# josedelrey/genetic-gaussian-splats

Measured on AMD Instinct MI355X. Metric: candidate renders/sec (and Gsplat-pixels/s), 512x512, 256 splats, pop=128, higher is better.
Workload: dtype fp32

## Files before the change

### genetic-gaussian-splats_amd/csrc/ggs_capi.cpp

```cpp
#include <hip/hip_runtime.h>
#include <math.h>
#include <stdarg.h>
#include <stdio.h>
#include <stdlib.h>
#include <string.h>

#include <algorithm>
#include <atomic>
#include <memory>
#include <mutex>
#include <string>
#include <vector>

#include "ggs_internal.h"


namespace ggs {
namespace {

thread_local std::string t_err;

int fail(int code, const char* fmt, ...) {
    char buf[512];
    va_list ap;
// ... 36 lines not shown
    }
    const size_t want = std::max<size_t>(bytes + bytes / 4, 4096);
    GGS_HIP(hipMalloc(&b.p, want));
    b.cap = want;
    return GGS_OK;
}

int ensure_zeroed(DevBuf& b, size_t bytes, hipStream_t st) {
    if (bytes <= b.cap) return GGS_OK;
    int rc = ensure(b, bytes, st);
    if (rc) return rc;
    GGS_HIP(hipMemsetAsync(b.p, 0, b.cap, st));
    return GGS_OK;
}

bool finalize_fused() {
    static const bool off = getenv("GGS_UNFUSED_FINALIZE") && atoi(getenv("GGS_UNFUSED_FINALIZE")) != 0;
    return !off;
}
bool fitness_api_fold() {
    const char* v = getenv("GGS_FITNESS_FOLD");
    return v && atoi(v) != 0;
}

struct PinBuf {
    void* p = nullptr;
    size_t cap = 0;
};

int ensure_pinned(PinBuf& b, size_t bytes) {
    if (bytes <= b.cap) return GGS_OK;
    if (b.p) {
        GGS_HIP(hipHostFree(b.p));
        b.p = nullptr;
        b.cap = 0;
    }
    const size_t want = std::max<size_t>(bytes + bytes / 4, 4096);
    GGS_HIP(hipHostMalloc(&b.p, want, hipHostMallocDefault));
    b.cap = want;
    return GGS_OK;
}

struct Workspace {
    hipStream_t stream = nullptr;
    DevBuf recs, bnds, partials, wpartials, order, plan, fctr;
    DevBuf maskws;
    int order_H = -1, order_W = -1;
    uint64_t plan_key = 0;
};

int ensure_tile_order(Workspace* w, int H, int W, hipStream_t st) {
    if (w->order_H == H && w->order_W == W) return GGS_OK;
    const int n = raster_order_len(H, W);
    int rc;
    if ((rc = ensure(w->order, sizeof(int) * (size_t)n, st))) return rc;
    std::vector<int> h(n);
    raster_tile_order(H, W, h.data());
#ifdef GGS_PROBE_BUILD
    if (const char* f = getenv("GGS_PROBE_ORDER")) {
        FILE* fp = fopen(f, "rb");
        if (!fp || fread(h.data(), sizeof(int), n, fp) != (size_t)n) {
            if (fp) fclose(fp);
            return fail(GGS_EINVAL, "GGS_PROBE_ORDER: cannot read the order");
        }
        fclose(fp);
    }
#endif
    GGS_HIP(hipStreamSynchronize(st));
    GGS_HIP(hipMemcpy(w->order.p, h.data(), sizeof(int) * n, hipMemcpyHostToDevice));
// ... 51 lines not shown
        if (!on) return;
        (void)hipEventRecord(b, st);
        std::lock_guard<std::mutex> lk(g_prof_mu);
        g_prof_pending.push_back({kernel, a, b});
    }
};

void prof_drain_locked() {
    for (auto& r : g_prof_pending) {
        float ms = 0.f;
        if (hipEventSynchronize(r.b) == hipSuccess && hipEventElapsedTime(&ms, r.a, r.b) == hipSuccess) {
            g_prof_ms[r.kernel] += ms;
            g_prof_n[r.kernel] += 1;
        }
        (void)hipEventDestroy(r.a);
        (void)hipEventDestroy(r.b);
    }
    g_prof_pending.clear();
}

int raster_fitness(hipStream_t st, int simds, const SplatRec* recs, const int4* bnds, int B, int N, int H, int W,
                   const float4* plan, float* partials, const float* wpartials, int mode, const int* order,
                   DevBuf& ctr, float* out, bool fuse, const unsigned char* dirty = nullptr,
                   const float* clean = nullptr, int group = 0) {
    const float bg[3] = {1.f, 1.f, 1.f};
    int nTX;
    const int nTiles = raster_tiles(H, W, &nTX);
    if (fuse && finalize_fused() && (4 * nTiles) % 32 == 0) {
        int rc;
        if ((rc = ensure_zeroed(ctr, sizeof(int) * (size_t)std::max(B, 1), st))) return rc;
        FinFused ff;
        ff.ctr = (int*)ctr.p;
        ff.wpartials = wpartials;
        ff.out = out;
        ff.hw = (double)H * (double)W;
        ff.mode = mode;
        ProfScope ps(st, 1);
        GGS_HIP(launch_raster(st, 1, recs, bnds, B, N, H, W, bg, nullptr, plan, partials, order, dirty, clean,
                              nullptr, &ff, simds, group));
        return GGS_OK;
    }
    {
        ProfScope ps(st, 1);
        GGS_HIP(launch_raster(st, 1, recs, bnds, B, N, H, W, bg, nullptr, plan, partials, order, dirty, clean,
                              nullptr, nullptr, simds, group));
    }
    ProfScope ps(st, 2);
    GGS_HIP(launch_finalize(st, partials, wpartials, B, nTiles, mode, H, W, out, nullptr, group));
    return GGS_OK;
}

struct DeviceGuard {
    int prev = -1;
    explicit DeviceGuard(int dev) {
        if (hipGetDevice(&prev) != hipSuccess) prev = -1;
        (void)hipSetDevice(dev);
    }
    ~DeviceGuard() {
        if (prev >= 0) (void)hipSetDevice(prev);
    }
};

struct StreamDrain {
    std::vector<std::pair<int, hipStream_t>> s;
    void add(int dev, hipStream_t st) {
        for (auto& x : s)
            if (x.second == st) return;
        s.emplace_back(dev, st);
// ... 99 lines not shown
    h ^= h >> 33;
    h *= P2;
    h ^= h >> 29;
    h *= P3;
    h ^= h >> 32;
    return h;
}

int check_dims(int64_t B, int32_t N, int32_t C, int32_t H, int32_t W) {
    if (B < 0 || N < 0) return fail(GGS_EINVAL, "B=%lld and N=%d must be >= 0", (long long)B, N);
    if (C < 9) return fail(GGS_EINVAL, "expected at least 9 genome cols, got C=%d (render.py:223)", C);
    if (H < 1 || W < 1) return fail(GGS_EINVAL, "H=%d, W=%d must be >= 1", H, W);
    if ((int64_t)N * (int64_t)sizeof(SplatRec) >= ((int64_t)1 << 31))
        return fail(GGS_EINVAL, "N=%d splats per candidate exceeds the limit %lld", N,
                    (long long)(((int64_t)1 << 31) / (int64_t)sizeof(SplatRec) - 1));
    int nTX;
    const int64_t nTiles = raster_tiles(H, W, &nTX);
    if (B * nTiles * 4 >= (int64_t)1 << 31)
        return fail(GGS_EINVAL, "B*tiles = %lld exceeds the grid limit; split the batch",
                    (long long)(B * nTiles * 4));
    return GGS_OK;
}

int run_fitness_planned(DevCtx* c, hipStream_t st, const float* d_gen, int64_t B, int N, int C,
                        const float4* plan, const float* wpartials, int mode, int H, int W, float k,
                        float* d_out, int group = 0);

int run_fitness(DevCtx* c, hipStream_t st, const float* d_gen, int64_t B, int N, int C,
                const float* d_target, const float* d_mask, int mode, float beta, int H, int W,
                float k, float* d_out, uint64_t plan_key = 0) {
    if (B == 0) return GGS_OK;
    Workspace* w = workspace_for(c, st);
    int nTX;
    const int nTiles = raster_tiles(H, W, &nTX);
    int rc;
    if ((rc = ensure(w->recs, sizeof(SplatRec) * (size_t)std::max<int64_t>(B * N, 1), st))) return rc;
    if ((rc = ensure(w->bnds, sizeof(int4) * (size_t)std::max<int64_t>(B * N, 1), st))) return rc;
    if ((rc = ensure(w->partials, sizeof(float) * 4 * (size_t)(B * nTiles), st))) return rc;
    if ((rc = ensure(w->wpartials, plan_wsum_bytes(H, W), st))) return rc;
    if ((rc = ensure_tile_order(w, H, W, st))) return rc;
    if (plan_key == 0 || plan_key != w->plan_key) {
        if ((rc = ensure(w->plan, plan_bytes(H, W), st))) return rc;
        GGS_HIP(launch_plan(st, d_target, d_mask, mode, beta, H, W, (float4*)w->plan.p,
                            (float*)w->wpartials.p));
        w->plan_key = plan_key;
    }
    return run_fitness_planned(c, st, d_gen, B, N, C, (const float4*)w->plan.p,
                               (const float*)w->wpartials.p, mode, H, W, k, d_out);
}

int run_fitness_planned(DevCtx* c, hipStream_t st, const float* d_gen, int64_t B, int N, int C,
                        const float4* plan, const float* wpartials, int mode, int H, int W, float k,
                        float* d_out, int group) {
    if (B == 0) return GGS_OK;
    Workspace* w = workspace_for(c, st);
    int nTX;
    const int nTiles = raster_tiles(H, W, &nTX);
    int rc;
    if ((rc = ensure(w->recs, sizeof(SplatRec) * (size_t)std::max<int64_t>(B * N, 1), st))) return rc;
    if ((rc = ensure(w->bnds, sizeof(int4) * (size_t)std::max<int64_t>(B * N, 1), st))) return rc;
    if ((rc = ensure(w->partials, sizeof(float) * 4 * (size_t)(B * nTiles), st))) return rc;
    if ((rc = ensure_tile_order(w, H, W, st))) return rc;
    SplatRec* recs = (SplatRec*)w->recs.p;
    {
        ProfScope ps(st, 0);
        GGS_HIP(launch_prep(st, true, d_gen, B * N, C, H, W, k, recs, (int4*)w->bnds.p, nullptr, nullptr, nullptr));
    }
    return raster_fitness(st, c->simds, recs, (const int4*)w->bnds.p, (int)B, N, H, W, plan, (float*)w->partials.p,
                          wpartials, mode, (const int*)w->order.p, w->fctr, d_out, fitness_api_fold(), nullptr,
                          nullptr, group);
}

int run_render(DevCtx* c, hipStream_t st, const float* d_gen, int64_t B, int N, int C, int H, int W,
               float k, const float bg[3], float* d_img) {
    if (B == 0) return GGS_OK;
    Workspace* w = workspace_for(c, st);
    int rc;
    if ((rc = ensure(w->recs, sizeof(SplatRec) * (size_t)std::max<int64_t>(B * N, 1), st))) return rc;
    if ((rc = ensure(w->bnds, sizeof(int4) * (size_t)std::max<int64_t>(B * N, 1), st))) return rc;
    if ((rc = ensure_tile_order(w, H, W, st))) return rc;
    SplatRec* recs = (SplatRec*)w->recs.p;
    {
        ProfScope ps(st, 0);
        GGS_HIP(launch_prep(st, false, d_gen, B * N, C, H, W, k, recs, (int4*)w->bnds.p, nullptr, nullptr, nullptr));
    }
    {
        ProfScope ps(st, 1);
        GGS_HIP(launch_raster(st, 0, recs, (const int4*)w->bnds.p, (int)B, N, H, W, bg, d_img, nullptr, nullptr,
                              (const int*)w->order.p, nullptr, nullptr, nullptr, nullptr, c->simds));
    }
    return GGS_OK;
}

void shard(int64_t B, int n, int d, int64_t* b0, int64_t* nb) {
    const int64_t per = (B + n - 1) / n;
    *b0 = std::min<int64_t>(B, d * per);
    *nb = std::min<int64_t>(B, *b0 + per) - *b0;
}

std::vector<int> g_comm_devs;
std::vector<void*> g_comms;

int local_comms_locked(const std::vector<DevCtx*>& cs, std::vector<void*>* out) {
    std::vector<int> devs;
    for (DevCtx* c : cs) devs.push_back(c->dev);
    if (devs != g_comm_devs) {
        for (void* c : g_comms) ggs_comm_destroy(c);
        g_comms.clear();
        g_comm_devs.clear();
        std::vector<void*> made(devs.size(), nullptr);
        const int rc = ggs_comm_init_local((int32_t)devs.size(), devs.data(), made.data());
        if (rc) return rc;
// ... 44 lines not shown
}

const char* ggs_last_error(void) { return t_err.c_str(); }

void ggs_shutdown(void) {
    {
        std::lock_guard<std::mutex> cl(g_comm_mu);
        for (void* c : g_comms) ggs_comm_destroy(c);
        g_comms.clear();
        g_comm_devs.clear();
    }
    std::lock_guard<std::mutex> lk(g_mu);
    {
        std::lock_guard<std::mutex> pl(g_prof_mu);
        prof_drain_locked();
    }
    for (auto& c : g_ctx) {
        if (!c) continue;
        std::lock_guard<std::mutex> cl(c->mu);
        (void)hipSetDevice(c->dev);
        (void)hipStreamSynchronize(c->stream);
        for (auto& w : c->ws) {
            if (w->stream) (void)hipStreamSynchronize(w->stream);
            for (DevBuf* b : {&w->recs, &w->bnds, &w->partials, &w->wpartials, &w->order, &w->plan, &w->fctr, &w->maskws})
                if (b->p) (void)hipFree(b->p);
        }
        for (DevBuf* b : {&c->gen, &c->out, &c->target, &c->mask, &c->prep_in, &c->prep_tgt, &c->prep_mask})
            if (b->p) (void)hipFree(b->p);
        for (PinBuf* b : {&c->h_out})
            if (b->p) (void)hipHostFree(b->p);
        (void)hipStreamDestroy(c->stream);
    }
    g_ctx.clear();
    g_active.clear();
    g_inited = false;
}

int ggs_fitness_device(int32_t device, void* stream, const float* d_genomes_axes, int64_t B, int32_t N,
                       int32_t C, const float* d_target_hw3, const float* d_mask_hw, int32_t mode,
                       float boost_beta, int32_t H, int32_t W, float k_sigma, float* d_out_B) {
    int rc = check_dims(B, N, C, H, W);
    if (rc) return rc;
    if (mode < GGS_FIT_NONE || mode > GGS_FIT_BOOST) return fail(GGS_EINVAL, "bad fitness mode %d", mode);
    if (mode != GGS_FIT_NONE && !d_mask_hw) return fail(GGS_EINVAL, "mode %d needs a weight mask", mode);
    if (B > 0 && (!d_genomes_axes && N > 0)) return fail(GGS_EINVAL, "null genomes");
    if (B > 0 && (!d_target_hw3 || !d_out_B)) return fail(GGS_EINVAL, "null target/out");
    DevCtx* c = nullptr;
// ... 2294 lines not shown
```

### genetic-gaussian-splats_amd/csrc/ggs_internal.h

```cpp
#pragma once
#include <hip/hip_runtime.h>
#include <stdint.h>

#include "../../include/ggs.h"

#if !defined(GGS_PROBE_BUILD) &&                                                         \
    (defined(GGS_NOPLAN) || defined(GGS_TIMING) || defined(GGS_VTIMING) || defined(GGS_SATURATE) || \
     defined(GGS_SAT_EVERY) || defined(GGS_SAT_BATCH) || defined(GGS_SAT_AHEAD) ||             \
     defined(GGS_CULL_AHEAD) || defined(GGS_CHUNK_MB) || defined(GGS_NO_RATIO_CLAMP) ||               \
     defined(GGS_DEPTH_SPLIT) || defined(GGS_TILE_H))
#error "GGS_* diagnostic knobs are for the probe build only: make probe PROBE=\"-D...\""
#endif
#ifdef GGS_PROBE_BUILD
#define GGS_BUILD_KIND "probe"
#else
#define GGS_BUILD_KIND "product"
#endif

namespace ggs {

struct __attribute__((aligned(16))) SplatRec {
    float C64, cx, r, cy8;
    float g, la, b, c128;
    float rho, rho4, A, B8;
    int x0, x1, y0, y1;
};
static_assert(sizeof(SplatRec) == 64, "SplatRec must be 64 bytes");

hipError_t launch_prep(hipStream_t st, bool encode, const float* genomes, int64_t S, int C, int H,
                       int W, float k, SplatRec* recs, int4* bnds, float* f9, int* i4, float* enc9,
                       const int* live = nullptr, int n_per = 0);
int raster_tiles(int H, int W, int* nTX);
struct FinFused {
    int* ctr = nullptr;
    const float* wpartials = nullptr;
    float* out = nullptr;
    double hw = 0.0;
    int mode = 0;
};
hipError_t launch_raster(hipStream_t st, int mode, const SplatRec* recs, const int4* bnds, int B, int N, int H, int W,
                         const float bg[3], float* img, const float4* plan, float* partials,
                         const int* tile_order, const unsigned char* dirty = nullptr,
                         const float* clean = nullptr, const int* live = nullptr, const FinFused* fin = nullptr,
                         int simds = 0, int group = 0);
int device_simds(int dev);

hipError_t launch_dirty(hipStream_t st, const float* curr, const float* nb, const SplatRec* cur_recs,
                        const SplatRec* nb_recs, int n, int N, int H, int W, unsigned char* dirty,
                        unsigned* n_changed, const int* live = nullptr, int rule = 1);
hipError_t launch_plan(hipStream_t st, const float* target, const float* mask, int mode, float beta,
                       int H, int W, float4* plan, float* wblock);
hipError_t launch_plan_set(hipStream_t st, const float* targets, const float* masks, int mode, float beta,
                           int H, int W, int K, float4* plans, float* wblocks);
size_t plan_bytes(int H, int W);
size_t plan_wsum_bytes(int H, int W);
void raster_tile_order(int H, int W, int* order);
int raster_order_len(int H, int W);
hipError_t launch_detmath(hipStream_t st, const float* x, const float* y, int64_t n, int fn,
                          float* out);
hipError_t launch_finalize(hipStream_t st, const float* partials, const float* wpartials, int B,
                           int nTiles, int mode, int H, int W, float* out, const int* live = nullptr,
                           int group = 0);

struct GaParamsDev {
    float sig_xy, sig_alog, sig_blog, sig_theta, sig_rgb, sig_alpha;
    float mutpb, cxpb;
    int tour_k;
// ... 212 lines not shown
```

### genetic-gaussian-splats_amd/csrc/ggs_kernels.hip

```cpp
#include <hip/hip_runtime.h>
#include <stdint.h>

#include <algorithm>
#include <atomic>
#include <utility>
#include <vector>

#include "ggs_detmath.h"
#include "ggs_internal.h"
#include "ggs_prep.h"

#if defined(__HIP_DEVICE_COMPILE__) && !defined(__gfx950__)
#error "ggs_kernels.hip targets gfx950 (MI355X) only"
#endif

namespace ggs {

using namespace detmath;

constexpr int PREP_THREADS = 64;
template <bool ENCODE>
__global__ void __launch_bounds__(PREP_THREADS)
prep_kernel(const float* __restrict__ genomes, int64_t S, int C, int H, int W, float k,
            SplatRec* __restrict__ recs, int4* __restrict__ bnds, float* __restrict__ f9, int* __restrict__ i4,
            float* __restrict__ enc9, const int* __restrict__ live, int n_per) {
    const int64_t i = (int64_t)blockIdx.x * blockDim.x + threadIdx.x;
    if (i >= S) return;
    if (live && i >= (int64_t)*live * n_per) return;
    const float* g = genomes + i * (int64_t)C;
    float row[9];
    if (ENCODE) {
        encode_row(g, row);
    } else {
#pragma unroll
        for (int j = 0; j < 9; ++j) row[j] = g[j];
    }
    if (enc9) {
#pragma unroll
        for (int j = 0; j < 9; ++j) enc9[i * 9 + j] = row[j];
    }
    const Prep13 p = preprocess_row(row, H, W, k);
    if (recs) {
        const SplatRec r = make_rec(p);
        recs[i] = r;
        bnds[i] = rec_bounds(r);
    }
    if (f9) {
        f9[0 * S + i] = p.cx;  f9[1 * S + i] = p.cy;  f9[2 * S + i] = p.sxx;
        f9[3 * S + i] = p.sxy; f9[4 * S + i] = p.syy; f9[5 * S + i] = p.rc;
        f9[6 * S + i] = p.gc;  f9[7 * S + i] = p.bc;  f9[8 * S + i] = p.a;
    }
    if (i4) {
        i4[0 * S + i] = p.x0; i4[1 * S + i] = p.x1; i4[2 * S + i] = p.y0; i4[3 * S + i] = p.y1;
    }
}

constexpr int TILE = 64;
#ifndef GGS_TILE_H
#define GGS_TILE_H 128
#endif
constexpr int TILE_H = GGS_TILE_H;
constexpr int RG = TILE_H / 4;
constexpr int NPK = RG / 2;
constexpr int WPB = 1;
constexpr int NT = 64 * WPB;
constexpr int SPB = 4 / WPB;
constexpr int CAP = 1024;
constexpr int OCC = 3;
// ... 10 lines not shown
#define GGS_NOPLAN 0
#endif

#ifndef GGS_SATURATE
#define GGS_SATURATE 1
#endif
constexpr float SAT_EPS = 5.9604645e-8f;
#ifndef GGS_SAT_EVERY
#define GGS_SAT_EVERY 16
#endif
constexpr int SAT_FIRST = 64, SAT_EVERY = GGS_SAT_EVERY;
constexpr int SAT_MIN_SPLATS = 512;
#ifndef GGS_SAT_BATCH
#define GGS_SAT_BATCH 384
#endif
#ifndef GGS_SAT_AHEAD
#define GGS_SAT_AHEAD 2
#endif
constexpr int SAT_BATCH = GGS_SAT_BATCH;

__device__ __forceinline__ int ufirst(int v) { return __builtin_amdgcn_readfirstlane(v); }

constexpr unsigned VW_ABOVE = 32u, VW_KA = 26, VW_CLIP = 31, VW_OFFSET = 0x03FFFFC0u;
__device__ __forceinline__ int visit_word(int i, const int4& bb, int ty0, int sx0) {
    constexpr int NP = GGS_TILE_H / 8;
    const int dy0 = bb.z - ty0, dy1 = bb.w - ty0;
    const unsigned kA = (unsigned)max(dy0, 0) >> 3;
    const unsigned kB = dy1 >= GGS_TILE_H - 1 ? (unsigned)NP : (unsigned)dy1 >> 3;
    const unsigned above = dy0 <= 0 ? VW_ABOVE : 0u;
    const unsigned clip = max(bb.x - sx0, sx0 + 15 - bb.y) > 0 ? (1u << VW_CLIP) : 0u;
    return (int)(((unsigned)i << 6) | kB | above | (kA << VW_KA) | clip);
}

__device__ __forceinline__ void store_partial(float* p, float v, bool fused) {
    if (fused) __hip_atomic_store(p, v, __ATOMIC_RELAXED, __HIP_MEMORY_SCOPE_AGENT);
    else *p = v;
}
__device__ __forceinline__ void strip_done(const FinFused& fin, const float* partials, int b, int nslots,
                                           int lane) {
    int old = 0;
    if (lane == 0) {
        asm volatile("s_waitcnt vmcnt(0)" ::: "memory");
        old = __hip_atomic_fetch_add(fin.ctr + b, 1, __ATOMIC_RELAXED, __HIP_MEMORY_SCOPE_AGENT);
    }
    if (ufirst(old) != nslots - 1) return;
    __builtin_amdgcn_fence(__ATOMIC_ACQUIRE, "agent");
    const float v = finalize_wave<true>(partials, fin.wpartials, nslots, fin.mode, fin.hw, b);
    if (lane == 0) {
        fin.out[b] = v;
        __hip_atomic_store(fin.ctr + b, 0, __ATOMIC_RELAXED, __HIP_MEMORY_SCOPE_AGENT);
    }
}

#ifndef GGS_TIMING
// ... 51 lines not shown
        P_T##k = P_T##k - w_;                                                        \
    } while (0)
#define GGS_BLEND_REC(k)                                                             \
    if ((k) < NPK) {                                                                 \
        F2 = F2 * R2;                                                                \
        R2 = R2 * (f2_t)s.rho;                                                       \
        GGS_BLEND(k, F2);                                                            \
    }
#if defined(GGS_NO_RATIO_CLAMP) && GGS_NO_RATIO_CLAMP
#define GGS_RATIO(qy8) GGS_EXP2(__builtin_fmaf((qy8), s.c128, abx.y))
#else
#define GGS_RATIO(qy8) GGS_EXP2(fminf(__builtin_fmaf((qy8), s.c128, abx.y), 100.0f))
#endif
#define GGS_E1(qy) ({                                                                     \
        f2_t t_, e2_, pxu_;                                                               \
        pxu_.x = px;                                                                      \
        const uint64_t ccp_ = *reinterpret_cast<const uint64_t*>(&s.C64);                  \
        asm("v_pk_fma_f32 %0, %1, %2, %3 op_sel:[0,0,1] op_sel_hi:[0,1,1]" : "=v"(t_) : "s"(ccp_), "v"(qy), "v"(abx)); \
        asm("v_pk_fma_f32 %0, %1, %2, %3 op_sel_hi:[1,1,0]" : "=v"(e2_) : "v"(qy), "v"(t_), "v"(pxu_)); \
        e2_; })
#define GGS_FOR8(X) X(0) X(1) X(2) X(3) X(4) X(5) X(6) X(7)
#define GGS_FOR16P(X) GGS_FOR8(X) X(8) X(9) X(10) X(11) X(12) X(13) X(14) X(15)

template <int MODE, bool SAT, bool FUSED, bool MULTI, bool LIST = false>
__device__ __forceinline__ void
raster_body(const SplatRec* __restrict__ recs, const int4* __restrict__ bnds, int B, int N, int H, int W, int nTX,
            int nTiles,
            float bg_r, float bg_g, float bg_b, float* __restrict__ img,
            const float4* __restrict__ plan, float* __restrict__ partials,
            const int* __restrict__ tile_order, const unsigned char* __restrict__ dirty,
            const float* __restrict__ clean, const int* __restrict__ live, int CH, FinFused fin, int simds,
            int group, const int* __restrict__ plan_of = nullptr) {
    static_assert(!MULTI || MODE == 1, "plan sets are for the fitness epilogue");
    static_assert(!LIST || MULTI, "a plan list names plans of a plan set");
    constexpr bool DS = GGS_DEPTH_SPLIT && MODE == 1 && !SAT;
    constexpr bool VW = !SAT && !FUSED;
    __shared__ int lists[DS ? 2 : WPB][CAP];

    const int lane = threadIdx.x & 63;
#if GGS_TIMING
    const unsigned long long rt_start = __builtin_amdgcn_s_memrealtime();
    unsigned long long t_cull = 0, t_vis = 0, t_mark = __builtin_amdgcn_s_memtime();
    unsigned n_vis = 0, n_done = 0;
#endif
#if GGS_DEPTH_SPLIT
    const int wib = DS ? 0 : ufirst((int)(threadIdx.x >> 6));
    const int half = DS ? ufirst((int)(threadIdx.x >> 6)) : 0;
#else
    const int wib = ufirst((int)(threadIdx.x >> 6));
#endif
    if (live) {
        B = ufirst(*live);
        if ((int64_t)blockIdx.x >= (int64_t)B * nTiles * SPB) return;
    }
    int idx = blockIdx.x, b0 = 0, Bc = B;
// ... 54 lines not shown
#else
    int* __restrict__ list = &lists[0][0] + wib * CAP;
#define GGS_NHI N
#define GGS_NLO 0
#define GGS_NR N
#define GGS_LIST_AT(q) list[q]
#endif
    const uint64_t lt_mask = (lane == 0) ? 0ull : (~0ull >> (64 - lane));
    int cnt = 0;
    auto saturated = [&]() __attribute__((always_inline)) {
        float m = 0.0f;
#define GGS_TMAX(k) if ((k) < NPK) m = fmaxf(m, fmaxf(P_T##k.x, P_T##k.y));
        GGS_FOR16P(GGS_TMAX)
#undef GGS_TMAX
        return !__ballot(m >= SAT_EPS);
    };

    auto bounds = [&](int i) { return cbnd[max(i, 0)]; };
#ifndef GGS_CULL_AHEAD
#define GGS_CULL_AHEAD 2
#endif
    constexpr int AHEAD = SAT ? GGS_SAT_AHEAD : GGS_CULL_AHEAD;
    static_assert(AHEAD >= 1 && AHEAD <= 4, "cull prefetch depth");
    int4 bbA = bounds(GGS_NHI - 1 - lane), bbB, bbC, bbD;
    if constexpr (AHEAD > 1) { __builtin_amdgcn_sched_barrier(0); bbB = bounds(GGS_NHI - 1 - lane - 64); }
    if constexpr (AHEAD > 2) { __builtin_amdgcn_sched_barrier(0); bbC = bounds(GGS_NHI - 1 - lane - 128); }
    if constexpr (AHEAD > 3) { __builtin_amdgcn_sched_barrier(0); bbD = bounds(GGS_NHI - 1 - lane - 192); }
    int base = 0;
    constexpr int LIMIT = SAT ? SAT_BATCH - 64 : CAP - 64 * AHEAD;
    static_assert(LIMIT + 64 * AHEAD <= CAP, "cull list capacity");
#if GGS_DEPTH_SPLIT
    for (int pass = 0;; ++pass) {
        if (DS ? pass > 0 : base >= nr) break;
#else
    while (base < N) {
#endif
        __builtin_amdgcn_s_setprio(CULL_PRIO);
#define GGS_CULL_CHUNK(BB)                                                                  \
        {                                                                                   \
            const int i = GGS_NHI - 1 - (base + lane);                                      \
            const int4 bb = BB;                                                \
            if (AHEAD == 1) BB = bounds(i - 64);                                            \
            const bool hit = (i >= GGS_NLO) & (bb.w >= ty0) & (bb.z <= ty1) & (bb.y >= sx0) & (bb.x <= sx0 + 15); \
                          \
            if (AHEAD > 1) BB = bounds(i - 64 * AHEAD);                                     \
            const uint64_t m = __ballot(hit);                                               \
            if (hit) list[cnt + __popcll(m & lt_mask)] =                                    \
                VW ? visit_word(i, bb, ty0, sx0) : i * (int)sizeof(SplatRec);                \
            cnt += __popcll(m);                                                             \
            base += 64;                                                                     \
        }
        if constexpr (AHEAD == 1) {
            GGS_CULL_CHUNK(bbA)
            if (cnt <= LIMIT && base < GGS_NR) continue;
        } else {
            do {
                GGS_CULL_CHUNK(bbA)
                GGS_CULL_CHUNK(bbB)
                if constexpr (AHEAD > 2) GGS_CULL_CHUNK(bbC)
                if constexpr (AHEAD > 3) GGS_CULL_CHUNK(bbD)
            } while (cnt <= LIMIT && base < GGS_NR);
        }
#undef GGS_CULL_CHUNK
#if GGS_DEPTH_SPLIT
        if constexpr (DS) {
            static_assert(!DS || SAT_MIN_SPLATS / 2 + 64 * AHEAD <= CAP, "depth split: one cull batch");
            if (lane == 0) s_cnt[half] = cnt;
            __syncthreads();
            c0 = ufirst(s_cnt[0]);
            const int total = c0 + ufirst(s_cnt[1]), hs = (total + 1) >> 1;
            lbase = half ? hs : 0;
            cnt = half ? total - hs : hs;
        }
#endif
        if (cnt == 0) continue;
// ... 345 lines not shown
    }
#if GGS_TIMING
    {
        GGS_TMARK(now);
        const unsigned long long rt_end = __builtin_amdgcn_s_memrealtime();
        if (lane == 0 && blockIdx.x < GGS_TIMING_WAVES) {
            unsigned long long* o = g_ggs_timing + 8 * (size_t)blockIdx.x;
            o[0] = rt_start; o[1] = rt_end; o[2] = t_cull; o[3] = t_vis; o[4] = now - t_mark;
            o[5] = (unsigned long long)__builtin_amdgcn_s_getreg(0xF804) |
                   ((unsigned long long)__builtin_amdgcn_s_getreg(0xF814) << 32);
            o[6] = n_vis; o[7] = n_done;
        }
    }
#endif
}

template <int MODE, bool SAT, bool FUSED>
__global__ void __launch_bounds__(GGS_DEPTH_SPLIT ? 2 * NT : NT, OCC)
raster_kernel(const SplatRec* __restrict__ recs, const int4* __restrict__ bnds, int B, int N, int H, int W, int nTX,
              int nTiles,
              float bg_r, float bg_g, float bg_b, float* __restrict__ img,
              const float4* __restrict__ plan, float* __restrict__ partials,
              const int* __restrict__ tile_order, const unsigned char* __restrict__ dirty,
              const float* __restrict__ clean, const int* __restrict__ live, int CH, FinFused fin, int simds) {
    raster_body<MODE, SAT, FUSED, false>(recs, bnds, B, N, H, W, nTX, nTiles, bg_r, bg_g, bg_b, img, plan, partials,
                                         tile_order, dirty, clean, live, CH, fin, simds, 1);
}

template <bool SAT, bool FUSED>
__global__ void __launch_bounds__(GGS_DEPTH_SPLIT ? 2 * NT : NT, OCC)
raster_multi_kernel(const SplatRec* __restrict__ recs, const int4* __restrict__ bnds, int B, int N, int H, int W,
                    int nTX, int nTiles, float bg_r, float bg_g, float bg_b, const float4* __restrict__ plan,
                    float* __restrict__ partials, const int* __restrict__ tile_order, int CH, FinFused fin,
                    int simds, int group) {
    raster_body<1, SAT, FUSED, true>(recs, bnds, B, N, H, W, nTX, nTiles, bg_r, bg_g, bg_b, nullptr, plan, partials,
                                     tile_order, nullptr, nullptr, nullptr, CH, fin, simds, group);
}

template <bool SAT>
__global__ void __launch_bounds__(GGS_DEPTH_SPLIT ? 2 * NT : NT, OCC)
chain_strips_kernel(const SplatRec* __restrict__ recs, const int4* __restrict__ bnds, int B, int N, int H, int W,
                    int nTX, int nTiles, float bg_r, float bg_g, float bg_b, const float4* __restrict__ plan,
                    float* __restrict__ partials, const int* __restrict__ tile_order,
                    const int* __restrict__ live, int CH, int simds, const int* __restrict__ plan_of) {
    raster_body<1, SAT, false, true, true>(recs, bnds, B, N, H, W, nTX, nTiles, bg_r, bg_g, bg_b, nullptr, plan,
                                           partials, tile_order, nullptr, nullptr, live, CH, FinFused{}, simds, 1,
                                           plan_of);
}

// ... 135 lines not shown
    const float a = x[i];
    float r, s, c;
    switch (fn) {
        case 0: r = det_expf(a); break;
        case 1: r = det_logf(a); break;
        case 2: det_sincosf(a, &s, &c); r = s; break;
        case 3: det_sincosf(a, &s, &c); r = c; break;
        case 4: r = ggs_sqrt_rn(a); break;
        default: r = ggs_div_rn(a, y[i]); break;
    }
    out[i] = r;
}

hipError_t launch_detmath(hipStream_t st, const float* x, const float* y, int64_t n, int fn,
                          float* out) {
    if (n <= 0) return hipSuccess;
    hipLaunchKernelGGL(detmath_kernel, dim3((unsigned)((n + 255) / 256)), dim3(256), 0, st, x, y, n,
                       fn, out);
    return hipGetLastError();
}

hipError_t launch_prep(hipStream_t st, bool encode, const float* genomes, int64_t S, int C, int H,
                       int W, float k, SplatRec* recs, int4* bnds, float* f9, int* i4, float* enc9, const int* live,
                       int n_per) {
    if (S <= 0) return hipSuccess;
    constexpr int PB = PREP_THREADS;
    const unsigned grid = (unsigned)((S + PB - 1) / PB);
    if (encode)
        hipLaunchKernelGGL(prep_kernel<true>, dim3(grid), dim3(PB), 0, st, genomes, S, C, H, W, k,
                           recs, bnds, f9, i4, enc9, live, n_per);
    else
        hipLaunchKernelGGL(prep_kernel<false>, dim3(grid), dim3(PB), 0, st, genomes, S, C, H, W, k,
                           recs, bnds, f9, i4, enc9, live, n_per);
    return hipGetLastError();
}

void raster_tile_order(int H, int W, int* order) {
    int nTX;
    const int n = raster_tiles(H, W, &nTX) * SPB;
    std::vector<std::pair<double, int>> d(n);
    for (int g = 0; g < n; ++g) {
        const int t = g / SPB, s = g % SPB;
        const double cx = (t % nTX) * TILE + (s + 0.5) * (TILE / SPB) - 0.5 * W;
        const double cy = (t / nTX) * TILE_H + 0.5 * TILE_H - 0.5 * H;
        d[g] = {cx * cx + cy * cy, g};
    }
    std::stable_sort(d.begin(), d.end());
    for (int g = 0; g < n; ++g) order[g] = d[g].second;
}

int raster_order_len(int H, int W) { return raster_tiles(H, W, nullptr) * SPB; }

int raster_tiles(int H, int W, int* nTX) {
    const int tx = (W + TILE - 1) / TILE, ty = (H + TILE_H - 1) / TILE_H;
    if (nTX) *nTX = tx;
    return tx * ty;
}

#ifndef GGS_CHUNK_MB
#define GGS_CHUNK_MB 40
#endif
constexpr int64_t CHUNK_BYTES = (int64_t)GGS_CHUNK_MB << 20;
int raster_chunk(int N) {
    const int64_t per = (int64_t)(N > 1 ? N : 1) * (int64_t)(sizeof(SplatRec) + sizeof(int4));
    int64_t ch = CHUNK_BYTES / per;
    if (ch > (1 << 24)) ch = 1 << 24;
    ch &= ~int64_t(7);
    return ch < 8 ? 8 : (int)ch;
}

int device_simds(int dev) {
    int cus = 0;
    if (hipDeviceGetAttribute(&cus, hipDeviceAttributeMultiprocessorCount, dev) != hipSuccess) return 0;
    return 4 * cus;
}

hipError_t launch_raster(hipStream_t st, int mode, const SplatRec* recs, const int4* bnds, int B, int N, int H, int W,
                         const float bg[3], float* img, const float4* plan, float* partials,
                         const int* tile_order, const unsigned char* dirty, const float* clean,
                         const int* live, const FinFused* fin, int simds, int group) {
    int nTX;
    const int nTiles = raster_tiles(H, W, &nTX);
    const dim3 grid((unsigned)((int64_t)B * nTiles * SPB)), block(NT);
    const bool sat = N > SAT_MIN_SPLATS;
    const dim3 block_f(GGS_DEPTH_SPLIT && !sat ? 2 * NT : NT);
    const int CH = raster_chunk(N);
    const FinFused ff = (mode != 0 && fin) ? *fin : FinFused{};
    if (GGS_DEPTH_SPLIT) simds = 0;
#define GGS_RASTER(M, S, F)                                                                    \
    hipLaunchKernelGGL((raster_kernel<M, S, F>), grid, (M) ? block_f : block, 0, st, recs, bnds, B, N, H, W, nTX, nTiles, \
                       bg[0], bg[1], bg[2], img, plan, partials, tile_order, dirty, clean, live, CH, ff, simds)
#define GGS_RASTER_MULTI(S, F)                                                                 \
    hipLaunchKernelGGL((raster_multi_kernel<S, F>), grid, block_f, 0, st, recs, bnds, B, N, H, W, nTX, nTiles, bg[0], \
                       bg[1], bg[2], plan, partials, tile_order, CH, ff, simds, group)
    if (group > 0) {
        if (mode != 1 || dirty || clean || live) return hipErrorInvalidValue;
        if (!ff.ctr) { if (!sat) GGS_RASTER_MULTI(false, false); else GGS_RASTER_MULTI(true, false); }
        else { if (!sat) GGS_RASTER_MULTI(false, true); else GGS_RASTER_MULTI(true, true); }
    }
    else if (mode == 0) { if (!sat) GGS_RASTER(0, false, false); else GGS_RASTER(0, true, false); }
    else if (!ff.ctr) { if (!sat) GGS_RASTER(1, false, false); else GGS_RASTER(1, true, false); }
    else { if (!sat) GGS_RASTER(1, false, true); else GGS_RASTER(1, true, true); }
#undef GGS_RASTER_MULTI
#undef GGS_RASTER
    return hipGetLastError();
}

hipError_t launch_chain_strips(hipStream_t st, const SplatRec* recs, const int4* bnds, int B, int N, int H, int W,
                               const float4* plans, float* partials, const int* tile_order, const int* live,
                               const int* plan_of, int simds) {
    int nTX;
    const int nTiles = raster_tiles(H, W, &nTX);
    if (!live || !plan_of) return hipErrorInvalidValue;
    const bool sat = N > SAT_MIN_SPLATS;
    const dim3 grid((unsigned)((int64_t)B * nTiles * SPB)), block(GGS_DEPTH_SPLIT && !sat ? 2 * NT : NT);
    const int CH = raster_chunk(N);
    if (GGS_DEPTH_SPLIT) simds = 0;
    if (!sat)
        hipLaunchKernelGGL(chain_strips_kernel<false>, grid, block, 0, st, recs, bnds, B, N, H, W, nTX, nTiles, 1.f,
                           1.f, 1.f, plans, partials, tile_order, live, CH, simds, plan_of);
    else
        hipLaunchKernelGGL(chain_strips_kernel<true>, grid, block, 0, st, recs, bnds, B, N, H, W, nTX, nTiles, 1.f,
                           1.f, 1.f, plans, partials, tile_order, live, CH, simds, plan_of);
    return hipGetLastError();
}
// ... 16 lines not shown
```

Before: 922,600.

## Precompute per-strip visit words and hit masks in prep for raster culling

The prep kernel now also builds, for each candidate, the per-tile-row visit words plus ballot-built 64-bit bitmasks. The masks record which splats touch each 16-pixel column strip, which ones it clips, and which touch each tile row. The unfused raster kernel then builds its per-tile cull list by ANDing these masks and scattering the precomputed words. This replaces loading each splat's bounds and testing them again in every tile. The cost is extra prep work, new workspace buffers and more memory traffic for the masks. Paths it does not cover (saturated, fused, depth-split, dirty or live) go to a bounds-culling kernel instead.

```diff
diff --git a/genetic-gaussian-splats_amd/csrc/ggs_capi.cpp b/genetic-gaussian-splats_amd/csrc/ggs_capi.cpp
--- a/genetic-gaussian-splats_amd/csrc/ggs_capi.cpp
+++ b/genetic-gaussian-splats_amd/csrc/ggs_capi.cpp
@@ -82,6 +82,10 @@
     const char* v = getenv("GGS_FITNESS_FOLD");
     return v && atoi(v) != 0;
 }
+bool strip_words_on() {
+    const char* v = getenv("GGS_STRIP_WORDS");
+    return !(v && *v && atoi(v) == 0);
+}
 
 struct PinBuf {
     void* p = nullptr;
@@ -105,6 +109,7 @@
     hipStream_t stream = nullptr;
     DevBuf recs, bnds, partials, wpartials, order, plan, fctr;
     DevBuf maskws;
+    DevBuf swords, smasks;
     int order_H = -1, order_W = -1;
     uint64_t plan_key = 0;
 };
@@ -202,7 +207,7 @@
 int raster_fitness(hipStream_t st, int simds, const SplatRec* recs, const int4* bnds, int B, int N, int H, int W,
                    const float4* plan, float* partials, const float* wpartials, int mode, const int* order,
                    DevBuf& ctr, float* out, bool fuse, const unsigned char* dirty = nullptr,
-                   const float* clean = nullptr, int group = 0) {
+                   const float* clean = nullptr, int group = 0, const StripWords& sw = StripWords{}) {
     const float bg[3] = {1.f, 1.f, 1.f};
     int nTX;
     const int nTiles = raster_tiles(H, W, &nTX);
@@ -223,7 +228,7 @@
     {
         ProfScope ps(st, 1);
         GGS_HIP(launch_raster(st, 1, recs, bnds, B, N, H, W, bg, nullptr, plan, partials, order, dirty, clean,
-                              nullptr, nullptr, simds, group));
+                              nullptr, nullptr, simds, group, sw));
     }
     ProfScope ps(st, 2);
     GGS_HIP(launch_finalize(st, partials, wpartials, B, nTiles, mode, H, W, out, nullptr, group));
@@ -369,6 +374,15 @@
     return GGS_OK;
 }
 
+int ensure_strip_words(Workspace* w, int64_t B, int N, int H, int W, hipStream_t st, StripWords* sw) {
+    if (!strip_words_ok(N) || !strip_words_on()) return GGS_OK;
+    int rc;
+    if ((rc = ensure(w->swords, strip_words_bytes(B, N, H, W), st))) return rc;
+    if ((rc = ensure(w->smasks, strip_masks_bytes(B, N, H, W), st))) return rc;
+    sw->words = (int*)w->swords.p;
+    sw->masks = (uint64_t*)w->smasks.p;
+    return GGS_OK;
+}
 int run_fitness_planned(DevCtx* c, hipStream_t st, const float* d_gen, int64_t B, int N, int C,
                         const float4* plan, const float* wpartials, int mode, int H, int W, float k,
                         float* d_out, int group = 0);
@@ -409,13 +423,17 @@
     if ((rc = ensure(w->partials, sizeof(float) * 4 * (size_t)(B * nTiles), st))) return rc;
     if ((rc = ensure_tile_order(w, H, W, st))) return rc;
     SplatRec* recs = (SplatRec*)w->recs.p;
+    const bool fold = fitness_api_fold();
+    StripWords sw;
+    if (group == 0 && !fold && (rc = ensure_strip_words(w, B, N, H, W, st, &sw))) return rc;
     {
         ProfScope ps(st, 0);
-        GGS_HIP(launch_prep(st, true, d_gen, B * N, C, H, W, k, recs, (int4*)w->bnds.p, nullptr, nullptr, nullptr));
+        GGS_HIP(launch_prep(st, true, d_gen, B * N, C, H, W, k, recs, (int4*)w->bnds.p, nullptr, nullptr, nullptr,
+                            nullptr, 0, sw, N));
     }
     return raster_fitness(st, c->simds, recs, (const int4*)w->bnds.p, (int)B, N, H, W, plan, (float*)w->partials.p,
-                          wpartials, mode, (const int*)w->order.p, w->fctr, d_out, fitness_api_fold(), nullptr,
-                          nullptr, group);
+                          wpartials, mode, (const int*)w->order.p, w->fctr, d_out, fold, nullptr,
+                          nullptr, group, sw);
 }
 
 int run_render(DevCtx* c, hipStream_t st, const float* d_gen, int64_t B, int N, int C, int H, int W,
@@ -427,14 +445,17 @@
     if ((rc = ensure(w->bnds, sizeof(int4) * (size_t)std::max<int64_t>(B * N, 1), st))) return rc;
     if ((rc = ensure_tile_order(w, H, W, st))) return rc;
     SplatRec* recs = (SplatRec*)w->recs.p;
+    StripWords sw;
+    if ((rc = ensure_strip_words(w, B, N, H, W, st, &sw))) return rc;
     {
         ProfScope ps(st, 0);
-        GGS_HIP(launch_prep(st, false, d_gen, B * N, C, H, W, k, recs, (int4*)w->bnds.p, nullptr, nullptr, nullptr));
+        GGS_HIP(launch_prep(st, false, d_gen, B * N, C, H, W, k, recs, (int4*)w->bnds.p, nullptr, nullptr, nullptr,
+                            nullptr, 0, sw, N));
     }
     {
         ProfScope ps(st, 1);
         GGS_HIP(launch_raster(st, 0, recs, (const int4*)w->bnds.p, (int)B, N, H, W, bg, d_img, nullptr, nullptr,
-                              (const int*)w->order.p, nullptr, nullptr, nullptr, nullptr, c->simds));
+                              (const int*)w->order.p, nullptr, nullptr, nullptr, nullptr, c->simds, 0, sw));
     }
     return GGS_OK;
 }
@@ -525,7 +546,8 @@
         (void)hipStreamSynchronize(c->stream);
         for (auto& w : c->ws) {
             if (w->stream) (void)hipStreamSynchronize(w->stream);
-            for (DevBuf* b : {&w->recs, &w->bnds, &w->partials, &w->wpartials, &w->order, &w->plan, &w->fctr, &w->maskws})
+            for (DevBuf* b : {&w->recs, &w->bnds, &w->partials, &w->wpartials, &w->order, &w->plan, &w->fctr, &w->maskws,
+                              &w->swords, &w->smasks})
                 if (b->p) (void)hipFree(b->p);
         }
         for (DevBuf* b : {&c->gen, &c->out, &c->target, &c->mask, &c->prep_in, &c->prep_tgt, &c->prep_mask})
diff --git a/genetic-gaussian-splats_amd/csrc/ggs_internal.h b/genetic-gaussian-splats_amd/csrc/ggs_internal.h
--- a/genetic-gaussian-splats_amd/csrc/ggs_internal.h
+++ b/genetic-gaussian-splats_amd/csrc/ggs_internal.h
@@ -27,9 +27,16 @@
 };
 static_assert(sizeof(SplatRec) == 64, "SplatRec must be 64 bytes");
 
+struct StripWords {
+    int* words = nullptr;
+    uint64_t* masks = nullptr;
+};
+bool strip_words_ok(int N);
+size_t strip_words_bytes(int64_t B, int N, int H, int W);
+size_t strip_masks_bytes(int64_t B, int N, int H, int W);
 hipError_t launch_prep(hipStream_t st, bool encode, const float* genomes, int64_t S, int C, int H,
                        int W, float k, SplatRec* recs, int4* bnds, float* f9, int* i4, float* enc9,
-                       const int* live = nullptr, int n_per = 0);
+                       const int* live = nullptr, int n_per = 0, const StripWords& sw = StripWords{}, int N = 0);
 int raster_tiles(int H, int W, int* nTX);
 struct FinFused {
     int* ctr = nullptr;
@@ -42,7 +49,7 @@
                          const float bg[3], float* img, const float4* plan, float* partials,
                          const int* tile_order, const unsigned char* dirty = nullptr,
                          const float* clean = nullptr, const int* live = nullptr, const FinFused* fin = nullptr,
-                         int simds = 0, int group = 0);
+                         int simds = 0, int group = 0, const StripWords& sw = StripWords{});
 int device_simds(int dev);
 
 hipError_t launch_dirty(hipStream_t st, const float* curr, const float* nb, const SplatRec* cur_recs,
diff --git a/genetic-gaussian-splats_amd/csrc/ggs_kernels.hip b/genetic-gaussian-splats_amd/csrc/ggs_kernels.hip
--- a/genetic-gaussian-splats_amd/csrc/ggs_kernels.hip
+++ b/genetic-gaussian-splats_amd/csrc/ggs_kernels.hip
@@ -19,12 +19,15 @@
 using namespace detmath;
 
 constexpr int PREP_THREADS = 64;
+__device__ __forceinline__ void prep_strip_words(int N, int H, int W, const int4& bb,
+                                                 int* __restrict__ swords, uint64_t* __restrict__ smasks);
 template <bool ENCODE>
 __global__ void __launch_bounds__(PREP_THREADS)
 prep_kernel(const float* __restrict__ genomes, int64_t S, int C, int H, int W, float k,
             SplatRec* __restrict__ recs, int4* __restrict__ bnds, float* __restrict__ f9, int* __restrict__ i4,
-            float* __restrict__ enc9, const int* __restrict__ live, int n_per) {
-    const int64_t i = (int64_t)blockIdx.x * blockDim.x + threadIdx.x;
+            float* __restrict__ enc9, const int* __restrict__ live, int n_per,
+            int* __restrict__ swords, uint64_t* __restrict__ smasks, int N) {
+    const int64_t i = (int64_t)blockIdx.x * blockDim.x + (smasks ? 63 - (int)threadIdx.x : (int)threadIdx.x);
     if (i >= S) return;
     if (live && i >= (int64_t)*live * n_per) return;
     const float* g = genomes + i * (int64_t)C;
@@ -44,6 +47,7 @@
         const SplatRec r = make_rec(p);
         recs[i] = r;
         bnds[i] = rec_bounds(r);
+        if (smasks) prep_strip_words(N, H, W, rec_bounds(r), swords, smasks);
     }
     if (f9) {
         f9[0 * S + i] = p.cx;  f9[1 * S + i] = p.cy;  f9[2 * S + i] = p.sxx;
@@ -100,14 +104,55 @@
 __device__ __forceinline__ int ufirst(int v) { return __builtin_amdgcn_readfirstlane(v); }
 
 constexpr unsigned VW_ABOVE = 32u, VW_KA = 26, VW_CLIP = 31, VW_OFFSET = 0x03FFFFC0u;
-__device__ __forceinline__ int visit_word(int i, const int4& bb, int ty0, int sx0) {
+__device__ __forceinline__ int visit_row_word(int i, const int4& bb, int ty0) {
     constexpr int NP = GGS_TILE_H / 8;
+    static_assert(NP == NPK, "kB counts the raster's packed row pairs");
+    static_assert(NPK < 32, "kB (0..NPK) lies below VW_ABOVE");
     const int dy0 = bb.z - ty0, dy1 = bb.w - ty0;
     const unsigned kA = (unsigned)max(dy0, 0) >> 3;
     const unsigned kB = dy1 >= GGS_TILE_H - 1 ? (unsigned)NP : (unsigned)dy1 >> 3;
     const unsigned above = dy0 <= 0 ? VW_ABOVE : 0u;
-    const unsigned clip = max(bb.x - sx0, sx0 + 15 - bb.y) > 0 ? (1u << VW_CLIP) : 0u;
-    return (int)(((unsigned)i << 6) | kB | above | (kA << VW_KA) | clip);
+    return (int)(((unsigned)i << 6) | kB | above | (kA << VW_KA));
+}
+__device__ __forceinline__ bool strip_clips(const int4& bb, int sx0) { return max(bb.x - sx0, sx0 + 15 - bb.y) > 0; }
+__device__ __forceinline__ int visit_word(int i, const int4& bb, int ty0, int sx0) {
+    return visit_row_word(i, bb, ty0) | (int)(strip_clips(bb, sx0) ? 1u << VW_CLIP : 0u);
+}
+static_assert(SAT_MIN_SPLATS * sizeof(SplatRec) <= VW_OFFSET + 64, "a record offset fits the word's offset field");
+
+__host__ __device__ constexpr int strip_mask_chunks(int N) { return ((N >> 6) + 3) & ~3; }
+__device__ __forceinline__ void prep_strip_words(int N, int H, int W, const int4& bb,
+                                                 int* __restrict__ swords, uint64_t* __restrict__ smasks) {
+    const int lane = threadIdx.x;
+    const int first = (int)(blockIdx.x * 64u), b = first / N, s = first - b * N + 63 - lane;
+    const int nTY = (H + TILE_H - 1) / TILE_H, nCS = (W + TILE - 1) / TILE * 4, R = 2 * nCS + nTY;
+    const int ncp = strip_mask_chunks(N);
+    for (int ty = 0; ty < nTY; ++ty) swords[((int64_t)b * nTY + ty) * N + s] = visit_row_word(s, bb, ty * TILE_H);
+    uint64_t* __restrict__ mcol = smasks + (int64_t)b * R * ncp + ((N >> 6) - 1 - (s >> 6));
+    const int lo = bb.x >> 4, hi = bb.y >> 4, flo = (bb.x + 15) >> 4, fhi = ((bb.y + 1) >> 4) - 1;
+    const int nW = (W + 15) >> 4;
+    for (int c0 = 0; c0 < nCS; c0 += 64) {
+        uint64_t mh = 0, mk = 0;
+        const int n = min(64, nW - c0);
+#pragma unroll 4
+        for (int j = 0; j < n; ++j) {
+            const int cs = c0 + j;
+            const uint64_t h = __builtin_amdgcn_ballot_w64((lo <= cs) & (cs <= hi));
+            const uint64_t k = __builtin_amdgcn_ballot_w64((cs < flo) | (cs > fhi));
+            const bool me = lane == j;
+            mh = me ? h : mh;
+            mk = me ? k : mk;
+        }
+        if (c0 + lane < nCS) {
+            mcol[(int64_t)(c0 + lane) * ncp] = mh;
+            mcol[(int64_t)(nCS + c0 + lane) * ncp] = mk;
+        }
+    }
+    for (int ty = 0; ty < nTY; ++ty) {
+        const int ty0 = ty * TILE_H, ty1 = min(ty0 + TILE_H, H) - 1;
+        const uint64_t m = __builtin_amdgcn_ballot_w64((bb.w >= ty0) & (bb.z <= ty1));
+        if (lane == 0) mcol[(int64_t)(2 * nCS + ty) * ncp] = m;
+    }
 }
 
 __device__ __forceinline__ void store_partial(float* p, float v, bool fused) {
@@ -205,7 +250,7 @@
 #define GGS_FOR8(X) X(0) X(1) X(2) X(3) X(4) X(5) X(6) X(7)
 #define GGS_FOR16P(X) GGS_FOR8(X) X(8) X(9) X(10) X(11) X(12) X(13) X(14) X(15)
 
-template <int MODE, bool SAT, bool FUSED, bool MULTI, bool LIST = false>
+template <int MODE, bool SAT, bool FUSED, bool MULTI, bool LIST = false, bool PRE = false>
 __device__ __forceinline__ void
 raster_body(const SplatRec* __restrict__ recs, const int4* __restrict__ bnds, int B, int N, int H, int W, int nTX,
             int nTiles,
@@ -213,7 +258,8 @@
             const float4* __restrict__ plan, float* __restrict__ partials,
             const int* __restrict__ tile_order, const unsigned char* __restrict__ dirty,
             const float* __restrict__ clean, const int* __restrict__ live, int CH, FinFused fin, int simds,
-            int group, const int* __restrict__ plan_of = nullptr) {
+            int group, const int* __restrict__ plan_of = nullptr, const int* __restrict__ swords = nullptr,
+            const uint64_t* __restrict__ smasks = nullptr) {
     static_assert(!MULTI || MODE == 1, "plan sets are for the fitness epilogue");
     static_assert(!LIST || MULTI, "a plan list names plans of a plan set");
     constexpr bool DS = GGS_DEPTH_SPLIT && MODE == 1 && !SAT;
@@ -314,10 +360,15 @@
 #endif
     constexpr int AHEAD = SAT ? GGS_SAT_AHEAD : GGS_CULL_AHEAD;
     static_assert(AHEAD >= 1 && AHEAD <= 4, "cull prefetch depth");
-    int4 bbA = bounds(GGS_NHI - 1 - lane), bbB, bbC, bbD;
-    if constexpr (AHEAD > 1) { __builtin_amdgcn_sched_barrier(0); bbB = bounds(GGS_NHI - 1 - lane - 64); }
-    if constexpr (AHEAD > 2) { __builtin_amdgcn_sched_barrier(0); bbC = bounds(GGS_NHI - 1 - lane - 128); }
-    if constexpr (AHEAD > 3) { __builtin_amdgcn_sched_barrier(0); bbD = bounds(GGS_NHI - 1 - lane - 192); }
+    static_assert(!PRE || (VW && !DS), "strip words are visit words");
+    constexpr bool pre = PRE;
+    int4 bbA = {}, bbB = {}, bbC = {}, bbD = {};
+    if constexpr (!pre) {
+        bbA = bounds(GGS_NHI - 1 - lane);
+        if constexpr (AHEAD > 1) { __builtin_amdgcn_sched_barrier(0); bbB = bounds(GGS_NHI - 1 - lane - 64); }
+        if constexpr (AHEAD > 2) { __builtin_amdgcn_sched_barrier(0); bbC = bounds(GGS_NHI - 1 - lane - 128); }
+        if constexpr (AHEAD > 3) { __builtin_amdgcn_sched_barrier(0); bbD = bounds(GGS_NHI - 1 - lane - 192); }
+    }
     int base = 0;
     constexpr int LIMIT = SAT ? SAT_BATCH - 64 : CAP - 64 * AHEAD;
     static_assert(LIMIT + 64 * AHEAD <= CAP, "cull list capacity");
@@ -342,7 +393,42 @@
             cnt += __popcll(m);                                                             \
             base += 64;                                                                     \
         }
-        if constexpr (AHEAD == 1) {
+        if constexpr (pre) {
+            static_assert(SAT_MIN_SPLATS <= LIMIT, "strip words: the whole cull is one batch");
+            const int nch = N >> 6, ncp = strip_mask_chunks(N), nTY = (H + TILE_H - 1) / TILE_H, nCS = nTX * 4;
+            const int ty = t / nTX;
+            const int* __restrict__ rw = swords + ((int64_t)b * nTY + ty) * N;
+            const uint64_t* __restrict__ mhit = smasks + ((int64_t)b * (2 * nCS + nTY) + (sx0 >> 4)) * ncp;
+            const uint64_t* __restrict__ mclip = mhit + (int64_t)nCS * ncp;
+            const uint64_t* __restrict__ mrow = mhit + (int64_t)(2 * nCS + ty - (sx0 >> 4)) * ncp;
+            for (int c0 = 0; c0 < nch; c0 += 4) {
+                const int i0 = N - 1 - 64 * c0 - lane;
+                int w0 = rw[i0], w1 = rw[max(i0 - 64, 0)], w2 = rw[max(i0 - 128, 0)], w3 = rw[max(i0 - 192, 0)];
+                uint64_t a0 = mhit[c0], a1 = mhit[c0 + 1], a2 = mhit[c0 + 2], a3 = mhit[c0 + 3];
+                uint64_t r0 = mrow[c0], r1 = mrow[c0 + 1], r2 = mrow[c0 + 2], r3 = mrow[c0 + 3];
+                uint64_t k0 = mclip[c0], k1 = mclip[c0 + 1], k2 = mclip[c0 + 2], k3 = mclip[c0 + 3];
+                asm volatile("" : "+v"(w0), "+v"(w1), "+v"(w2), "+v"(w3), "+s"(a0), "+s"(a1), "+s"(a2), "+s"(a3),
+                                  "+s"(r0), "+s"(r1), "+s"(r2), "+s"(r3), "+s"(k0), "+s"(k1), "+s"(k2), "+s"(k3));
+                const uint64_t h0 = a0 & r0;
+                const uint64_t h1 = a1 & r1 & (c0 + 1 < nch ? ~0ull : 0ull);
+                const uint64_t h2 = a2 & r2 & (c0 + 2 < nch ? ~0ull : 0ull);
+                const uint64_t h3 = a3 & r3 & (c0 + 3 < nch ? ~0ull : 0ull);
+#define GGS_LIST_CHUNK(WD, HM, KM)                                                              \
+                {                                                                           \
+                    if (__builtin_amdgcn_inverse_ballot_w64(HM))                            \
+                        list[cnt + (int)__builtin_amdgcn_mbcnt_hi((unsigned)((HM) >> 32),   \
+                                        __builtin_amdgcn_mbcnt_lo((unsigned)(HM), 0u))] =   \
+                            __builtin_amdgcn_inverse_ballot_w64(KM) ? (WD) | (int)(1u << VW_CLIP) : (WD); \
+                    cnt += __popcll(HM);                                                    \
+                }
+                GGS_LIST_CHUNK(w0, h0, k0)
+                GGS_LIST_CHUNK(w1, h1, k1)
+                GGS_LIST_CHUNK(w2, h2, k2)
+                GGS_LIST_CHUNK(w3, h3, k3)
+#undef GGS_LIST_CHUNK
+            }
+            base = N;
+        } else if constexpr (AHEAD == 1) {
             GGS_CULL_CHUNK(bbA)
             if (cnt <= LIMIT && base < GGS_NR) continue;
         } else {
@@ -734,9 +820,23 @@
               float bg_r, float bg_g, float bg_b, float* __restrict__ img,
               const float4* __restrict__ plan, float* __restrict__ partials,
               const int* __restrict__ tile_order, const unsigned char* __restrict__ dirty,
-              const float* __restrict__ clean, const int* __restrict__ live, int CH, FinFused fin, int simds) {
-    raster_body<MODE, SAT, FUSED, false>(recs, bnds, B, N, H, W, nTX, nTiles, bg_r, bg_g, bg_b, img, plan, partials,
-                                         tile_order, dirty, clean, live, CH, fin, simds, 1);
+              const float* __restrict__ clean, const int* __restrict__ live, int CH, FinFused fin, int simds,
+              const int* __restrict__ swords, const uint64_t* __restrict__ smasks) {
+    constexpr bool PRE = !SAT && !FUSED && !GGS_DEPTH_SPLIT;
+    raster_body<MODE, SAT, FUSED, false, false, PRE>(recs, bnds, B, N, H, W, nTX, nTiles, bg_r, bg_g, bg_b, img, plan,
+                                                     partials, tile_order, dirty, clean, live, CH, fin, simds, 1,
+                                                     nullptr, swords, smasks);
+}
+
+template <int MODE>
+__global__ void __launch_bounds__(GGS_DEPTH_SPLIT ? 2 * NT : NT, OCC)
+bounds_cull_kernel(const SplatRec* __restrict__ recs, const int4* __restrict__ bnds, int B, int N, int H, int W,
+                   int nTX, int nTiles, float bg_r, float bg_g, float bg_b, float* __restrict__ img,
+                   const float4* __restrict__ plan, float* __restrict__ partials,
+                   const int* __restrict__ tile_order, const unsigned char* __restrict__ dirty,
+                   const float* __restrict__ clean, const int* __restrict__ live, int CH, int simds) {
+    raster_body<MODE, false, false, false>(recs, bnds, B, N, H, W, nTX, nTiles, bg_r, bg_g, bg_b, img, plan, partials,
+                                           tile_order, dirty, clean, live, CH, FinFused{}, simds, 1);
 }
 
 template <bool SAT, bool FUSED>
@@ -918,16 +1018,19 @@
 
 hipError_t launch_prep(hipStream_t st, bool encode, const float* genomes, int64_t S, int C, int H,
                        int W, float k, SplatRec* recs, int4* bnds, float* f9, int* i4, float* enc9, const int* live,
-                       int n_per) {
+                       int n_per, const StripWords& sw, int N) {
     if (S <= 0) return hipSuccess;
+    const bool strips = sw.masks && sw.words && recs && !live && strip_words_ok(N) && S % N == 0 && S < ((int64_t)1 << 31);
+    int* const swords = strips ? sw.words : nullptr;
+    uint64_t* const smasks = strips ? sw.masks : nullptr;
     constexpr int PB = PREP_THREADS;
     const unsigned grid = (unsigned)((S + PB - 1) / PB);
     if (encode)
         hipLaunchKernelGGL(prep_kernel<true>, dim3(grid), dim3(PB), 0, st, genomes, S, C, H, W, k,
-                           recs, bnds, f9, i4, enc9, live, n_per);
+                           recs, bnds, f9, i4, enc9, live, n_per, swords, smasks, N);
     else
         hipLaunchKernelGGL(prep_kernel<false>, dim3(grid), dim3(PB), 0, st, genomes, S, C, H, W, k,
-                           recs, bnds, f9, i4, enc9, live, n_per);
+                           recs, bnds, f9, i4, enc9, live, n_per, swords, smasks, N);
     return hipGetLastError();
 }
 
@@ -947,6 +1050,15 @@
 
 int raster_order_len(int H, int W) { return raster_tiles(H, W, nullptr) * SPB; }
 
+bool strip_words_ok(int N) { return N > 0 && N <= SAT_MIN_SPLATS && N % 64 == 0; }
+size_t strip_words_bytes(int64_t B, int N, int H, int W) {
+    return sizeof(int) * (size_t)B * (size_t)((H + TILE_H - 1) / TILE_H) * (size_t)N;
+}
+size_t strip_masks_bytes(int64_t B, int N, int H, int W) {
+    const size_t rows = 2 * (size_t)((W + TILE - 1) / TILE) * 4 + (size_t)((H + TILE_H - 1) / TILE_H);
+    return sizeof(uint64_t) * (size_t)B * rows * (size_t)strip_mask_chunks(N);
+}
+
 int raster_tiles(int H, int W, int* nTX) {
     const int tx = (W + TILE - 1) / TILE, ty = (H + TILE_H - 1) / TILE_H;
     if (nTX) *nTX = tx;
@@ -974,7 +1086,7 @@
 hipError_t launch_raster(hipStream_t st, int mode, const SplatRec* recs, const int4* bnds, int B, int N, int H, int W,
                          const float bg[3], float* img, const float4* plan, float* partials,
                          const int* tile_order, const unsigned char* dirty, const float* clean,
-                         const int* live, const FinFused* fin, int simds, int group) {
+                         const int* live, const FinFused* fin, int simds, int group, const StripWords& sw) {
     int nTX;
     const int nTiles = raster_tiles(H, W, &nTX);
     const dim3 grid((unsigned)((int64_t)B * nTiles * SPB)), block(NT);
@@ -983,20 +1095,30 @@
     const int CH = raster_chunk(N);
     const FinFused ff = (mode != 0 && fin) ? *fin : FinFused{};
     if (GGS_DEPTH_SPLIT) simds = 0;
+    const bool strips = !GGS_DEPTH_SPLIT && sw.masks && sw.words && !live && !dirty && strip_words_ok(N);
+    const int* const swords = strips ? sw.words : nullptr;
+    const uint64_t* const smasks = strips ? sw.masks : nullptr;
 #define GGS_RASTER(M, S, F)                                                                    \
     hipLaunchKernelGGL((raster_kernel<M, S, F>), grid, (M) ? block_f : block, 0, st, recs, bnds, B, N, H, W, nTX, nTiles, \
-                       bg[0], bg[1], bg[2], img, plan, partials, tile_order, dirty, clean, live, CH, ff, simds)
+                       bg[0], bg[1], bg[2], img, plan, partials, tile_order, dirty, clean, live, CH, ff, simds, swords, smasks)
 #define GGS_RASTER_MULTI(S, F)                                                                 \
     hipLaunchKernelGGL((raster_multi_kernel<S, F>), grid, block_f, 0, st, recs, bnds, B, N, H, W, nTX, nTiles, bg[0], \
                        bg[1], bg[2], plan, partials, tile_order, CH, ff, simds, group)
+#define GGS_BOUNDS_CULL(M)                                                                     \
+    hipLaunchKernelGGL((bounds_cull_kernel<M>), grid, (M) ? block_f : block, 0, st, recs, bnds, B, N, H, W, nTX, nTiles, \
+                       bg[0], bg[1], bg[2], img, plan, partials, tile_order, dirty, clean, live, CH, simds)
     if (group > 0) {
         if (mode != 1 || dirty || clean || live) return hipErrorInvalidValue;
         if (!ff.ctr) { if (!sat) GGS_RASTER_MULTI(false, false); else GGS_RASTER_MULTI(true, false); }
         else { if (!sat) GGS_RASTER_MULTI(false, true); else GGS_RASTER_MULTI(true, true); }
     }
-    else if (mode == 0) { if (!sat) GGS_RASTER(0, false, false); else GGS_RASTER(0, true, false); }
-    else if (!ff.ctr) { if (!sat) GGS_RASTER(1, false, false); else GGS_RASTER(1, true, false); }
+    else if (mode == 0) {
+        if (sat) GGS_RASTER(0, true, false); else if (strips) GGS_RASTER(0, false, false); else GGS_BOUNDS_CULL(0);
+    } else if (!ff.ctr) {
+        if (sat) GGS_RASTER(1, true, false); else if (strips) GGS_RASTER(1, false, false); else GGS_BOUNDS_CULL(1);
+    }
     else { if (!sat) GGS_RASTER(1, false, true); else GGS_RASTER(1, true, true); }
+#undef GGS_BOUNDS_CULL
 #undef GGS_RASTER_MULTI
 #undef GGS_RASTER
     return hipGetLastError();
```

Result: faster. 933,400, median of 6 (+1.2%).
